# tiems90/mosaic

Hardware: AMD Instinct MI355X
Metric: PIP-join points/sec (H3 res 9) at 1/2/4/8 GPUs + achieved HBM GB/s (higher is better)
Workload: dtype f64

## Files before the change

mosaic_amd/csrc/capi.cpp:

```cpp
#include <hip/hip_runtime.h>

#include <algorithm>
#include <unordered_map>
#include <unordered_set>
#include <chrono>
#include <sched.h>
#include <array>
#include <atomic>
#include <cmath>
#include <cstdarg>
#include <cstdio>
#include <cstring>
#include <cstdlib>
#include <limits>
#include <string>
#include <map>
#include <memory>
#include <functional>
#include <tuple>
#include <mutex>
#include <thread>
#include <vector>

#include "../../include/mosaic_arrow.h"
// ... 1507 lines not shown
  std::vector<uint64_t> ref(ties.size());
  mgpu::parallel_for((int64_t)ties.size(), 256, [&](int64_t b, int64_t e, int) {
    for (int64_t k = b; k < e; k++)
      ref[k] = cells ? mgpu::h3glibc::point_to_cell(ties[k].x, ties[k].y, res)
                     : mgpu::h3glibc::lattice_key(ties[k].x, ties[k].y, res);
  });
  std::vector<std::pair<int64_t, uint64_t>> diff;
  for (size_t k = 0; k < ties.size(); k++)
    if (ref[k] != ties[k].key) diff.push_back({ties[k].pos, ref[k]});
  std::sort(diff.begin(), diff.end());
  return diff;
}

int32_t check_res(int32_t is, int32_t res) {
  if (is == MGPU_H3) {
    if (res < 0 || res > 15) return fail(MGPU_E_RESOLUTION, "H3 resolution has to be between 0 and 15; found %d", res);
    return MGPU_OK;
  }
  if (is == MGPU_BNG) {
    if (res == 0 || res < -6 || res > 6) return fail(MGPU_E_RESOLUTION, "BNG resolution not supported; found %d", res);
    return MGPU_OK;
  }
  return fail(MGPU_E_INVALID_ARG, "unknown index system %d (0 = H3, 1 = BNG)", is);
}

int32_t set_device(int dev) {
  HIP_TRY(hipSetDevice(dev));
  return MGPU_OK;
}

}

extern "C" {

const char* mgpu_last_error(void) { return g_err.c_str(); }
const char* mgpu_version(void) { return "mosaic-mi355x 0.1.0 (gfx950)"; }
int32_t mgpu_join_tile_points(void) { return (int32_t)mgpu::join_tile_points(); }

int32_t mgpu_check_resolution(int32_t index_system, int32_t res) { return check_res(index_system, res); }

int32_t mgpu_ctx_create(int32_t device_id, mgpu_ctx** out) {
  if (!out) return fail(MGPU_E_INVALID_ARG, "out is NULL");
  int n = 0;
  HIP_TRY(hipGetDeviceCount(&n));
  if (device_id < 0 || device_id >= n) return fail(MGPU_E_INVALID_ARG, "device %d not present (%d GPUs)", device_id, n);
  HIP_TRY(hipSetDevice(device_id));
  mgpu_ctx* c = new mgpu_ctx();
  c->device = device_id;
  int32_t st = MGPU_OK;
  if (hipEventCreate(&c->ev0) != hipSuccess || hipEventCreate(&c->ev1) != hipSuccess ||
      hipEventCreate(&c->ev2) != hipSuccess || hipEventCreate(&c->ev3) != hipSuccess ||
      hipHostMalloc((void**)&c->pin, kPinWords * 8, hipHostMallocDefault) != hipSuccess)
    st = fail(MGPU_E_DEVICE, "mgpu_ctx_create: events / pinned page");
  if (!st) st = ensure_ws(c, 1);
  if (!st) st = ensure_tq(c, kTqInit);
  if (st) {
    mgpu_ctx_destroy(c);
    return st;
  }
  *out = c;
  return MGPU_OK;
}

int32_t mgpu_ctx_destroy(mgpu_ctx* ctx) {
  if (!ctx) return MGPU_OK;
  mgpu_comm_destroy(ctx);
  hipSetDevice(ctx->device);
  if (ctx->split_ws) hipFree(ctx->split_ws);
  if (ctx->bin_ws) hipFree(ctx->bin_ws);
  if (ctx->scratch) hipFree(ctx->scratch);
  if (ctx->redo) hipFree(ctx->redo);
  if (ctx->tq) hipFree(ctx->tq);
  if (ctx->ovr) hipFree(ctx->ovr);
  if (ctx->ws) hipFree(ctx->ws);
  if (ctx->pin) hipHostFree(ctx->pin);
  if (ctx->ev0) hipEventDestroy(ctx->ev0);
  if (ctx->ev1) hipEventDestroy(ctx->ev1);
  if (ctx->ev2) hipEventDestroy(ctx->ev2);
  if (ctx->ev3) hipEventDestroy(ctx->ev3);
  delete ctx;
  return MGPU_OK;
}

int32_t mgpu_ctx_set_option(mgpu_ctx* ctx, const char* key, int64_t v) {
  if (!ctx || !key) return fail(MGPU_E_INVALID_ARG, "ctx/key is NULL");
  mgpu_options& o = ctx->opt;
  const std::string k = key;
  auto bad = [&]() { return fail(MGPU_E_INVALID_ARG, "option %s: value %lld out of range", key, (long long)v); };
  if (k == "h3_libm") {
    if (v != MGPU_LIBM_REFERENCE && v != MGPU_LIBM_CORRECTLY_ROUNDED) return bad();
    o.h3_libm = v;
  } else if (k == "pipeline") {
    if (v < MGPU_PIPELINE_AUTO || v > MGPU_PIPELINE_BINNED) return bad();
    o.pipeline = v;
  } else if (k == "bin_count") {
    if (v < 1 || v > mgpu::bin_max()) return bad();
    o.bin_count = v;
  } else if (k == "bin_min_mb") {
    if (v < 0) return bad();
    o.bin_min_mb = v;
  } else if (k == "bin_min_points") {
    if (v < 0) return bad();
    o.bin_min_points = v;
  } else if (k == "bin_xcd") {
    if (v != 0 && v != 1) return bad();
    o.bin_xcd = v;
// ... 1234 lines not shown
    return fail(MGPU_E_INVALID_ARG, "chip table lives on device %d, context on device %d", chips->device, ctx->device);
  if (n < 0 || (n > 0 && (!x || !y))) return fail(MGPU_E_INVALID_ARG, "bad point arrays");
  if (capacity < 0 || (capacity > 0 && (!out_point || !out_poly))) return fail(MGPU_E_INVALID_ARG, "bad output arrays");
  if (int32_t st = set_device(ctx->device)) return st;
  int64_t tiles = mgpu::join_tiles(n);
  const bool emit = count_pool < 0;
  const int64_t pool = emit ? capacity : count_pool;
  if (int32_t st = ensure_ws(ctx, tiles, pool)) return st;
  auto* base = (uint8_t*)ctx->ws;
  const WsLayout L = ws_layout(tiles, pool);
  const mgpu_options& o = ctx->opt;
  mgpu::JoinArgs a;
  a.x = x;
  a.y = y;
  a.n = n;
  a.n_tiles = tiles;
  a.res = res;
  a.res_match = (is == MGPU_BNG || chips->view.res < 0 || chips->view.res == res) ? 1 : 0;
  a.chips = chips->view;
  a.counters = (unsigned long long*)base;
  a.pool_used = a.counters + 5;
  a.n_dirty = (uint32_t*)(a.counters + 6);
  a.dirty = (uint32_t*)(base + L.dirty);
  a.pool_cap = pool;
  a.tile_count = (uint32_t*)(base + L.count);
  a.tile_where = (uint64_t*)(base + L.where);
  a.recs = (uint64_t*)(base + L.recs);
  a.tie_queue = ctx->tq;
  a.tie_cap = ctx->tq_cap;
  a.ovr = ctx->ovr;
  a.n_ovr = n_ovr;
  a.tie_host = (is == MGPU_H3 && tie_host) ? 1 : 0;
  a.pos_of = nullptr;
  mgpu::EmitArgs e;
  e.tile_count = a.tile_count;
  e.group_off = (uint64_t*)(base + L.off);
  a.group_sum = (uint32_t*)(base + L.gsum);
  a.group_cand = a.group_sum + (tiles / 32 + 1);
  e.tile_where = a.tile_where;
  e.recs = a.recs;
  e.point_id = point_id;
  e.id_base = id_base;
  e.capacity = capacity;
  e.out_point = out_point;
  e.out_poly = out_poly;
  a.valid = valid;
  a.valid_off = valid_off;
  a.mixed_idx = nullptr;
  a.mixed_res = nullptr;
  a.chunk_mixed = nullptr;
  a.extra = nullptr;
  a.n_extra = nullptr;
  a.poly_answers = 0;
  HIP_TRY(hipMemsetAsync(base, 0, kWsCounters, s));
  HIP_TRY(hipMemsetAsync(ctx->tq, 0, 16, s));
  const bool bng_grid = is == MGPU_BNG && chips->view.raster_mode == mgpu::kRasterNone &&
                        chips->view.probe_mode == mgpu::kProbeDense && o.bng_split;
  const bool split = (o.pipeline == MGPU_PIPELINE_AUTO || o.pipeline == MGPU_PIPELINE_SPLIT) && n > 0 &&
                     (chips->view.raster_mode != mgpu::kRasterNone || bng_grid) && a.res_match &&
                     (is == MGPU_H3 || res == chips->view.res) && chips->view.max_cell_chips <= 32;
  mgpu::SplitArgs sa{};
  if (split) {
    const int64_t nc = mgpu::split_chunks(n), C = mgpu::split_chunk();
    size_t off = 0;
    auto carve = [&](size_t bytes) {
      const size_t o_ = off;
      off = align_up(off + bytes, 256);
      return o_;
    };
    const size_t o_codes = carve((size_t)nc * C * 4), o_idx = carve((size_t)nc * C * 2), o_res = carve((size_t)nc * C * 8);
    const size_t o_pairs = carve(nc * 4), o_mixed = carve(nc * 4), o_cand = carve(nc * 4), o_off = carve(nc * 8);
    const size_t o_extra = carve((size_t)nc * (C / mgpu::join_tile_points()) * 4);
    if (off > ctx->split_bytes) {
      if (ctx->split_ws) HIP_TRY(hipFree(ctx->split_ws));
      ctx->split_ws = nullptr;
      ctx->split_bytes = 0;
      HIP_TRY(hipMalloc(&ctx->split_ws, off));
      ctx->split_bytes = off;
    }
    auto* sb = (uint8_t*)ctx->split_ws;
    sa.codes = sb + o_codes;
    sa.mixed_idx = (uint16_t*)(sb + o_idx);
    sa.chunk_pairs = (uint32_t*)(sb + o_pairs);
    sa.chunk_mixed = (uint32_t*)(sb + o_mixed);
    sa.chunk_off = (uint64_t*)(sb + o_off);
    a.extra = sa.extra = (uint32_t*)(sb + o_extra);
    a.n_extra = (uint32_t*)(a.counters + 7);
    a.group_sum = sa.chunk_pairs;
    a.group_cand = (uint32_t*)(sb + o_cand);
    a.mixed_idx = sa.mixed_idx;
    a.mixed_res = (uint64_t*)(sb + o_res);
    a.chunk_mixed = sa.chunk_mixed;
    sa.point_id = point_id;
    sa.id_base = id_base;
    sa.capacity = capacity;
    sa.out_point = out_point;
    sa.out_poly = out_poly;
    sa.j = a;
    HIP_TRY(hipMemsetAsync(a.group_cand, 0, nc * 4, s));
  }
  mgpu::BinArgs ba{};
  const bool binned = !split && plan_bins(o, chips, is, res, n, valid, a, ba);
  if (binned) {
    const int64_t nc = mgpu::split_chunks(n), C = mgpu::split_chunk();
    const int64_t K = mgpu::bin_chunks(n), G = mgpu::bin_groups(n), nb = (int64_t)ba.nbx * ba.nby;
    size_t off = 0;
    auto carve = [&](size_t bytes) {
      const size_t o_ = off;
      off = align_up(off + bytes, 256);
      return o_;
    };
    const size_t o_perm = carve((size_t)n * 4), o_rorig = carve((size_t)n * 8);
    const size_t o_bx = carve((size_t)n * 8), o_by = carve((size_t)n * 8),
                 o_pre = carve((size_t)K * nb * 4), o_res = carve((size_t)nc * C * 8), o_cnt = carve((size_t)K * nb * 4),
                 o_gs = carve((size_t)G * nb * 4), o_pairs = carve(nc * 4), o_off = carve(nc * 8),
                 o_gperm = carve(nc * 4), o_gcand = carve(nc * 4);
    const mgpu::ChipTableView& cv = chips->view;
    uint64_t grid_entries = 0;
    for (int f = 0; f < 20; f++) grid_entries = std::max<uint64_t>(grid_entries, (uint64_t)cv.dense[f].base + (uint64_t)cv.dense[f].w * cv.dense[f].h);
    const bool keyed = is == MGPU_H3 && cv.probe_mode == mgpu::kProbeDense && o.bin_keys && grid_entries < (1ull << 30);
    const size_t o_key = keyed ? carve((size_t)n * 4) : 0;
    if (off > ctx->bin_bytes) {
      if (ctx->bin_ws) HIP_TRY(hipFree(ctx->bin_ws));
      ctx->bin_ws = nullptr;
      ctx->bin_bytes = 0;
      HIP_TRY(hipMalloc(&ctx->bin_ws, off));
      ctx->bin_bytes = off;
    }
    auto* bb = (uint8_t*)ctx->bin_ws;
    ba.x = x;
    ba.y = y;
    ba.bx = (double*)(bb + o_bx);
    ba.by = (double*)(bb + o_by);
    ba.pre = (uint32_t*)(bb + o_pre);
    ba.perm = (uint32_t*)(bb + o_perm);
    ba.res = (uint64_t*)(bb + o_rorig);
    ba.cnt = (uint32_t*)(bb + o_cnt);
    ba.gsum = (uint32_t*)(bb + o_gs);
    ba.key = keyed ? (uint32_t*)(bb + o_key) : nullptr;
    mgpu::JoinArgs j = a;
    j.bin_key = ba.key;
    j.x = ba.bx;
    j.y = ba.by;
    j.mixed_idx = nullptr;
    j.chunk_mixed = nullptr;
    j.poly_answers = 1;
    j.pos_of = ba.perm;
    j.mixed_res = (uint64_t*)(bb + o_res);
    j.group_sum = (uint32_t*)(bb + o_gperm);
    j.group_cand = (uint32_t*)(bb + o_gcand);
    ba.s.j = j;
    ba.s.chunk_pairs = (uint32_t*)(bb + o_pairs);
// ... 109 lines not shown
  if (!L.valid || L.binned || (!L.split && pool_used > 0)) return launch_call(ctx, c, timed, n_ovr, 0);
  const int64_t unit = L.split ? mgpu::split_chunk() : mgpu::join_tile_points();
  const int64_t n_units = L.split ? mgpu::split_chunks(L.n) : L.n_tiles;
  std::vector<uint32_t> list;
  for (int64_t p : pos)
    if (list.empty() || list.back() != (uint32_t)(p / unit)) list.push_back((uint32_t)(p / unit));
  if ((int64_t)list.size() * (L.split ? mgpu::split_chunk_tiles() : 1) > L.n_tiles)
    return launch_call(ctx, c, timed, n_ovr, 0);
  const size_t o_aff = 256, o_list = align_up(o_aff + (size_t)n_units, 256), o_old = o_list + list.size() * 4;
  const size_t bytes = o_old + list.size() * 4;
  if (bytes > ctx->redo_bytes) {
    if (ctx->redo) HIP_TRY(hipFree(ctx->redo));
    ctx->redo = nullptr;
    ctx->redo_bytes = 0;
    HIP_TRY(hipMalloc(&ctx->redo, bytes));
    ctx->redo_bytes = bytes;
  }
  auto* rb = (uint8_t*)ctx->redo;
  mgpu::RedoArgs R{(const uint32_t*)(rb + o_list), (uint32_t*)(rb + o_old), rb + o_aff, (uint32_t*)rb,
                   (uint32_t*)(rb + 4)};
  mgpu::JoinArgs a = L.split ? L.sargs.j : L.jargs;
  a.ovr = ctx->ovr;
  a.n_ovr = n_ovr;
  a.tie_host = 0;
  HIP_TRY(hipMemsetAsync(rb, 0, o_list, c.s));
  HIP_TRY(hipMemsetAsync(rb + 4, 0xFF, 4, c.s));
  HIP_TRY(hipMemcpyAsync(rb + o_list, list.data(), list.size() * 4, hipMemcpyHostToDevice, c.s));
  const uint32_t nd = L.split ? 0u : (uint32_t)list.size();
  HIP_TRY(hipMemcpyAsync(a.n_dirty, &nd, 4, hipMemcpyHostToDevice, c.s));
  HIP_TRY(hipStreamSynchronize(c.s));
  if (L.split) {
    mgpu::SplitArgs sa = L.sargs;
    sa.j = a;
    HIP_TRY(mgpu::launch_split_redo(c.is, sa, R, (int64_t)list.size(), c.s, c.count_pool < 0));
    L.sargs = sa;
  } else {
    HIP_TRY(mgpu::launch_join_redo(c.is, a, L.emit, R, (int64_t)list.size(), c.s, c.count_pool < 0));
    L.jargs = a;
  }
  if (timed) HIP_TRY(hipEventRecord(ctx->ev1, c.s));
  if (c.d_n_pairs) HIP_TRY(hipMemcpyAsync(c.d_n_pairs, ctx->ws, 8, hipMemcpyDeviceToDevice, c.s));
  L.n_ovr = n_ovr;
  L.tie_host = 0;
  return MGPU_OK;
}

static int32_t settle_join(mgpu_ctx* ctx, const JoinCall& c, bool timed, bool reference_libm, int64_t* out_n_pairs,
                           mgpu_stats* stats) {
  const hipStream_t s = c.s;
  int64_t n_ovr = 0, n_ties = 0, n_moved = 0;
  int overflows = 0;
  uint64_t h[8] = {0};
  for (;;) {
    HIP_TRY(hipMemcpyAsync(ctx->pin, ctx->ws, 16 * 8, hipMemcpyDeviceToHost, s));
    HIP_TRY(hipMemcpyAsync(ctx->pin + 16, ctx->tq, (2 + 4 * kTqHead) * 8, hipMemcpyDeviceToHost, s));
    HIP_TRY(stream_wait(ctx, s));
    memcpy(h, ctx->pin, sizeof h);
    const int64_t queued = (int64_t)ctx->pin[16];
    if (h[2]) break;
    if (queued > ctx->tq_cap) {
      if (++overflows > 2) return fail(MGPU_E_INTERNAL, "pip_join: the near-tie queue overflowed %d times", overflows);
      if (int32_t e = ensure_tq(ctx, queued + queued / 4 + 1024)) return e;
      if (int32_t e = launch_call(ctx, c, timed, n_ovr, reference_libm && n_ovr == 0)) return e;
      continue;
    }
    if (n_ovr > 0) break;
    n_ties = queued;
    if (!reference_libm || n_ties == 0) break;
    std::vector<TieRec> tr;
    if (int32_t e = read_ties(ctx, n_ties, tr)) return e;
    const auto ref = libm_reference_keys(tr, c.res);
    n_moved = 0;
    for (size_t k = 0; k < tr.size(); k++) n_moved += ref[k].second != tr[k].key;
    if (n_moved == 0) break;
    std::vector<uint64_t> hv(2 * ref.size());
    for (size_t k = 0; k < ref.size(); k++) hv[2 * k] = (uint64_t)ref[k].first, hv[2 * k + 1] = ref[k].second;
    if (int32_t e = ensure_ovr(ctx, (int64_t)hv.size())) return e;
    HIP_TRY(hipMemcpy(ctx->ovr, hv.data(), hv.size() * 8, hipMemcpyHostToDevice));
    n_ovr = (int64_t)ref.size();
    std::vector<int64_t> pos(ref.size());
    for (size_t k = 0; k < ref.size(); k++) pos[k] = (int64_t)ref[k].first;
    if (int32_t e = launch_override_pass(ctx, c, timed, n_ovr, pos, h[5])) return e;
  }
  const int32_t is = c.is;
  const int64_t n = c.n, capacity = c.capacity;
  if (out_n_pairs) *out_n_pairs = (int64_t)h[0];
  if (stats) {
    stats->n_points = n;
    stats->n_pairs = (int64_t)h[0];
    stats->n_near_ties = n_ties;
    stats->n_candidates = (int64_t)h[3];
    stats->libm_overrides = (int32_t)n_moved;
    float ms = 0, ms2 = 0;
    if (timed) {
      hipEventElapsedTime(&ms, ctx->ev0, ctx->ev1);
      if (n > 0) hipEventElapsedTime(&ms2, ctx->ev0, ctx->ev2);
    }
    stats->kernel_ms = ms;
    stats->stream_kernel_ms = ms2;
    stats->mixed_kernel_ms = stats->emit_kernel_ms = 0;
    if (!timed) {
    } else if (ctx->last.split && n > 0) {
      float m3 = 0;
      hipEventElapsedTime(&m3, ctx->ev0, ctx->ev3);
      stats->mixed_kernel_ms = m3 - ms2;
      stats->emit_kernel_ms = ms - m3;
    } else if (ctx->last.binned && n > 0) {
      float m3 = 0;
// ... 667 lines not shown
```

mosaic_amd/csrc/capi_internal.h:

```cpp
#pragma once
#include <hip/hip_runtime.h>
#include <stdint.h>

#include "../../include/mosaic_gpu.h"
#include "chip_table.h"
#include "kernels.h"

struct mgpu_options {
  int64_t h3_libm = MGPU_LIBM_REFERENCE;
  int64_t pipeline = MGPU_PIPELINE_AUTO;
  int64_t bin_count = 64;
  int64_t bin_min_mb = 256;
  int64_t bin_min_points = 1 << 21;
  int64_t bin_xcd = 1;
  int64_t bin_keys = 0;
  int64_t spin_us = 2000;
  int64_t ring_batch = (int64_t)1 << 26;
  int64_t count_lds_slots = 4096;
  int64_t count_groups = 0;
  int64_t kring_batch = 0;
  int64_t bng_split = 0;
  int64_t raster = 1, raster_bng = 0, raster_sub = 16, raster_milli = 250;
};

struct mgpu_ctx {
  int device = 0;
  mgpu_options opt;
  void* ws = nullptr;
  size_t ws_bytes = 0;
  hipEvent_t ev0 = nullptr, ev1 = nullptr, ev2 = nullptr, ev3 = nullptr;
  void* comm = nullptr;
  void* split_ws = nullptr;
  size_t split_bytes = 0;
  void* bin_ws = nullptr;
  size_t bin_bytes = 0;
  uint64_t* tq = nullptr;
  int64_t tq_cap = 0;
  uint64_t* ovr = nullptr;
  int64_t ovr_cap = 0;
  uint64_t* pin = nullptr;
  void* scratch = nullptr;
  size_t scratch_bytes = 0;
  void* redo = nullptr;
  size_t redo_bytes = 0;
  struct {
    bool valid = false, pool_ok = false;
    const mgpu_chips* chips = nullptr;
    int32_t is = 0, res = 0;
    const double *x = nullptr, *y = nullptr;
    const int64_t* point_id = nullptr;
    int64_t id_base = 0, n = 0, total = 0;
    const uint8_t* pts_valid = nullptr;
    int64_t pts_valid_off = 0;
    mgpu::EmitArgs emit{};
    mgpu::JoinArgs jargs{};
    int64_t n_tiles = 0;
    int64_t n_ovr = 0;
    int tie_host = 0;
    bool split = false;
    mgpu::SplitArgs sargs{};
    bool binned = false;
    mgpu::BinArgs bargs{};
    bool async_pending = false;
    int64_t* d_n_pairs = nullptr;
    void* stream = nullptr;
    int64_t capacity = 0;
    int64_t* out_point = nullptr;
    int32_t* out_poly = nullptr;
    int64_t pool = 0, pool_used = 0;
  } last;
};

struct mgpu_chips {
  int device = 0;
  int32_t index_system = MGPU_H3;
  void* blob = nullptr;
  size_t bytes = 0;
  mgpu::ChipTableView view{};
  int64_t n_vertices = 0;
  mutable void* slots = nullptr;
};

namespace mgpu {
int32_t set_error(int32_t code, const char* fmt, ...);
int64_t blob_bytes_of_header(const void* header);
constexpr int64_t kBlobHeaderSize = 1024;
int32_t adopt_device_blob(mgpu_ctx* ctx, void* dev_blob, int64_t bytes, mgpu_chips** out);
}
```

mosaic_amd/csrc/kernels.h:

```cpp
#pragma once
#include <hip/hip_runtime.h>
#include <stdint.h>

#include "../../include/mosaic_gpu.h"
#include "chip_table.h"

namespace mgpu {

struct JoinArgs {
  const double* x;
  const double* y;
  int64_t n;
  int64_t n_tiles;
  int res;
  int res_match;
  ChipTableView chips;
  uint32_t* tile_count;
  uint32_t* group_sum;
  uint32_t* group_cand;
  uint64_t* tile_where;
  uint64_t* recs;
  int64_t pool_cap;
  unsigned long long* pool_used;
  uint32_t* dirty;
// ... 44 lines not shown
};
int64_t split_chunk();
int64_t split_chunk_tiles();
int64_t split_chunks(int64_t n);
hipError_t launch_split(int is, const SplitArgs& a, hipStream_t s, hipEvent_t after_classify, hipEvent_t after_mixed,
                        bool emit = true);
hipError_t launch_split_emit(int is, const SplitArgs& a, hipStream_t s);
hipError_t launch_split_redo(int is, const SplitArgs& sa, const RedoArgs& R, int64_t n, hipStream_t s,
                             bool emit = true);

struct BinArgs {
  SplitArgs s;
  const double* x;
  const double* y;
  double* bx;
  double* by;
  uint32_t* perm;
  uint64_t* res;
  uint32_t* cnt;
  uint32_t* pre;
  uint32_t* gsum;
  double x0, y0, inv_bx, inv_by;
  int32_t nbx, nby;
  int32_t xcd_runs;
  uint32_t* key;
};
int64_t bin_chunk();
int64_t bin_chunks(int64_t n);
int64_t bin_groups(int64_t n);
int32_t bin_max();
hipError_t launch_binned(int is, const BinArgs& a, hipStream_t s, hipEvent_t after_bin, hipEvent_t after_join,
                         bool emit = true);
hipError_t launch_bin_emit(const BinArgs& a, hipStream_t s);

struct EmitArgs {
  const uint32_t* tile_count;
  uint64_t* group_off;
  const uint64_t* tile_where;
  const uint64_t* recs;
  const int64_t* point_id;
  int64_t id_base;
  int64_t capacity;
  int64_t* out_point;
  int32_t* out_poly;
  const uint32_t* redo_first = nullptr;
  const uint8_t* redo_affected = nullptr;
};


hipError_t launch_cells(int is, int res, const double* x, const double* y, int64_t n, int64_t* out,
                        unsigned long long* counters, unsigned long long* ties, int64_t tie_cap,
                        uint64_t* tie_queue, int64_t tq_cap, hipStream_t s, const uint8_t* valid = nullptr,
                        int64_t voff = 0);
hipError_t launch_scatter_i64(const int64_t* pos, const int64_t* val, int64_t n, int64_t* out, hipStream_t s);
hipError_t launch_gather_xy(const double* x, const double* y, const int64_t* pos, int64_t n, double* xy,
                            hipStream_t s);
hipError_t launch_decode_internal(const int32_t* type_id, const int64_t* row_part, const int64_t* part_ring,
                                  const int64_t* ring_off, const double* xy, const uint8_t* valid, int64_t voff,
                                  int64_t n, double* x, double* y, unsigned long long* counters, hipStream_t s);
hipError_t launch_decode_points(int format, const uint8_t* data, const void* offsets, int off32, const uint8_t* valid,
                                int64_t voff, int64_t n, double* x, double* y, unsigned long long* counters,
                                hipStream_t s);
hipError_t launch_valid_and(const uint8_t* a, int64_t aoff, const uint8_t* b, int64_t boff, int64_t n, uint8_t* out,
                            hipStream_t s);
int64_t join_tiles(int64_t n);
int64_t join_tile_points();
int64_t join_slot_records();
hipError_t launch_join(int is, const JoinArgs& a, const EmitArgs& e, hipStream_t s, hipEvent_t after_stream,
                       bool emit = true);
hipError_t launch_join_redo(int is, const JoinArgs& a, const EmitArgs& e, const RedoArgs& R, int64_t n, hipStream_t s,
                            bool emit = true);
hipError_t launch_emit(const EmitArgs& e, int64_t n_tiles, hipStream_t s);

struct CountArgs {
  const int32_t* ids;
  uint32_t n_slots;
  const uint32_t* chip_slot;
  const uint32_t* dense;
  int32_t min_id;
  uint32_t contiguous;
  uint32_t lds_slots;
  uint32_t hash_slots;
  uint32_t stage_n;
  const int64_t* weight;
  unsigned long long* count;
  unsigned long long* sum;
  uint32_t* dropped;
  uint32_t max_groups;
};
constexpr int64_t kCountLdsSlotsMax = 4096;
constexpr int64_t kCountGroupsMax = 65536;
constexpr uint32_t kCountHash = 4096;
constexpr int64_t kCountStageMax = 2048;
hipError_t launch_split_count(int is, const SplitArgs& a, const CountArgs& c, hipStream_t s);
hipError_t launch_tile_count(const EmitArgs& e, int64_t n_tiles, const CountArgs& c, hipStream_t s);
hipError_t launch_bin_count(const BinArgs& b, const CountArgs& c, hipStream_t s);
int64_t format_chunks(int64_t n);
hipError_t launch_format_cells(int is, const int64_t* cells, int64_t n, char* out, int64_t out_bytes,
                               int64_t* offsets, int64_t* chunk, unsigned long long* counters, hipStream_t s);
int64_t format_chunks(int64_t n);
hipError_t launch_kring_count(int is, const int64_t* cells, int64_t n, int k, int loop_only, int64_t* mc,
                              int64_t* chunk, uint32_t* fb_idx, unsigned long long* counters, hipStream_t s);
int64_t kring_fallback_words(int k);
int32_t kring_fallback_max_k();
hipError_t launch_kring_fallback(const int64_t* cells, const uint32_t* fb_idx, int64_t j0, int64_t j1, int k,
                                 int loop_only, int64_t* mc, int64_t* chunk, const int64_t* offsets, int64_t* out,
// ... 9 lines not shown
```

mosaic_amd/csrc/kernels.hip:

```cpp
#include <hip/hip_runtime.h>
#include <stdint.h>

#include <map>
#include <mutex>

#define H3T_QUAL static __constant__ const
#include "h3_core.h"
#include "bng_core.h"
#include "pip_core.h"
#include "h3_ring.h"
#include "kernels.h"
#include "raster.h"

namespace mgpu {

#ifndef MGPU_BLOCK
#define MGPU_BLOCK 64
#endif
constexpr int kBlock = MGPU_BLOCK;
constexpr int kItems = 4;
constexpr int kTile = kBlock * kItems;
constexpr int kStreamBlock = 256;
static_assert(kTile <= 1024, "point-in-tile indices are 10 bits");

// ... 1184 lines not shown
      for (int k = 0; k < kCfyBatch; k++) {
#if MGPU_CFY_ABLATE == 1
        cl[k] = ri[k] < kRasterFull ? (ri[k] & 1) : kPixEmpty;
#elif MGPU_CFY_ABLATE == 2
        cl[k] = ri[k] < kRasterFull && bi[k] != kNoPixel && s_blk[bi[k]] != kPixMixed ? s_blk[bi[k]] : kPixEmpty;
#elif MGPU_CFY_ABLATE == 3
        cl[k] = ri[k] < kRasterFull ? (bi[k] != kNoPixel && s_blk[bi[k]] != kPixMixed ? s_blk[bi[k]] : t.raster[ri[k]])
                                    : kPixEmpty;
#elif MGPU_CFY_ABLATE == 4
        cl[k] = ri[k] < kRasterFull ? t.raster[ri[k]] : kPixEmpty;
#elif MGPU_CFY_ABLATE == 5
        cl[k] = ri[k] < kRasterFull ? (bi[k] != kNoPixel && s_blk[bi[k]] != kPixMixed ? s_blk[bi[k]] : kPixMixed)
                                    : kPixEmpty;
#else
        if (IS == MGPU_BNG && bng_grid)
          cl[k] = ri[k] == kRasterFull ? kPixMixed : (ri[k] == kNoPixel ? kPixEmpty : ri[k]);
        else
          cl[k] = ri[k] < kRasterFull ? raster_class_blk(t, s_blk, ri[k], bi[k], sb[k], s_band)
                                      : (ri[k] == kRasterFull ? kPixMixed : kPixEmpty);
#endif
        if (IS == MGPU_BNG && bng_grid) ge[k] = gix[k];
        else ge[k] = (IS == MGPU_BNG && ri[k] < kRasterFull) ? t.grid[gix[k]] : 0ull;
      }
#pragma unroll
      for (int k = 0; k < kCfyBatch; k++) {
        const int64_t p = c0 + (int64_t)(b + k) * 64 + lane;
        const bool valid = p < a.n;
        bool mixed = cl[k] == kPixMixed;
        Code code;
        if (IS == MGPU_H3) {
          code = (Code)cl[k];
          if (!mixed && cl[k] != kPixEmpty) {
            const uint32_t c = cl[k];
            pairs += c < t.raster_pc[0] ? 1u : c < t.raster_pc[1] ? 2u : c < t.raster_pc[2] ? 3u : c < t.raster_pc[3] ? 4u
                     : (uint32_t)__popc((uint32_t)(t.raster_cls[c] >> 32));
          }
        } else {
          const uint32_t first = (uint32_t)ge[k], m = cl[k];
          if (!mixed && m && !(m < 256u && first < (1u << 24))) mixed = true;
          code = (Code)(mixed ? kCodeMixed32 : (m ? (first << 8) | m : 0u));
          if (!mixed) pairs += __popc(m);
        }
        if (valid) MGPU_ST_INTER(code, &codes[p]);
        mixed = mixed && valid;
        const unsigned long long bal = __ballot(mixed);
        if (mixed) sa.mixed_idx[c0 + nmixed + (uint32_t)__popcll(bal & below)] = (uint16_t)((b + k) * 64 + lane);
        nmixed += (uint32_t)__popcll(bal);
      }
    }
    pairs = wave_sum_u32(pairs);
    if (lane == 0) {
      sa.chunk_pairs[ch] = pairs;
      sa.chunk_mixed[ch] = nmixed;
    }
  }
  count_wave(&a.counters[2], any_bad);
}


#ifndef MGPU_CFY_PAIR
#define MGPU_CFY_PAIR 1
#endif
typedef double dbl2_t __attribute__((ext_vector_type(2)));
template <int IS>
__global__ __launch_bounds__(kCfyBlock) __attribute__((amdgpu_waves_per_eu(MGPU_CFY_WAVES))) void classify_pair_kernel(SplitArgs sa, int64_t n_chunks) {
  using Code = typename CodeOf<IS>::T;
  constexpr int kW = kCfyBlock / 64;
  constexpr int kPairItems = kChunk / 128;
  constexpr int kPB = kCfyBatch / 2 > 0 ? kCfyBatch / 2 : 1;
  constexpr int kPts = 2 * kPB;
  static_assert(kPairItems % kPB == 0, "MGPU_CFY_BATCH / 2 must divide the pair items per lane of a chunk");
  const JoinArgs& a = sa.j;
  const ChipTableView& t = a.chips;
  extern __shared__ uint16_t s_blk[];
  const int lane = threadIdx.x & 63, wave = threadIdx.x >> 6;
  const bool use_blk = IS == MGPU_H3 && t.raster_blk != nullptr;
  const bool bng_grid = IS == MGPU_BNG && t.raster_mode == kRasterNone;
  const uint32_t nblk = use_blk ? t.raster_bnx * t.raster_bny : 0u;
  uint32_t* s_band = (uint32_t*)(s_blk + ((nblk + 1) & ~1u));
  if (use_blk)
    for (uint32_t i = threadIdx.x; i < nblk; i += kCfyBlock) s_blk[i] = t.raster_blk[i];
  if (IS == MGPU_H3)
    for (uint32_t i = threadIdx.x; i < t.raster_nband; i += kCfyBlock) s_band[i] = t.raster_band[i];
  __syncthreads();
  Code* codes = (Code*)sa.codes;
  const unsigned long long below = (1ull << lane) - 1ull;
  bool any_bad = false;
  const int64_t ch_step = (int64_t)gridDim.x * kW;
  for (int64_t ch = (int64_t)blockIdx.x * kW + wave; ch < n_chunks; ch += ch_step) {
    const int64_t c0 = ch * kChunk;
    uint32_t pairs = 0, nmixed = 0;
    for (int b = 0; b < kPairItems; b += kPB) {
      double X[kPts], Y[kPts];
#pragma unroll
      for (int k = 0; k < kPB; k++) {
        const int64_t p = c0 + (int64_t)(b + k) * 128 + 2 * lane;
        if (p + 1 < a.n) {
          const dbl2_t vx = __builtin_nontemporal_load((const dbl2_t*)(a.x + p));
          const dbl2_t vy = __builtin_nontemporal_load((const dbl2_t*)(a.y + p));
          X[2 * k] = vx.x, X[2 * k + 1] = vx.y, Y[2 * k] = vy.x, Y[2 * k + 1] = vy.y;
        } else {
          X[2 * k] = Y[2 * k] = X[2 * k + 1] = Y[2 * k + 1] = 0.0;
          if (p < a.n) X[2 * k] = a.x[p], Y[2 * k] = a.y[p];
        }
      }
      uint32_t ri[kPts], gix[kPts], sb[kPts], bi[kPts];
// ... 31 lines not shown
                                      : (ri[j] == kRasterFull ? kPixMixed : kPixEmpty);
          ge[j] = (IS == MGPU_BNG && ri[j] < kRasterFull) ? t.grid[gix[j]] : 0ull;
        }
      }
      Code code[kPts];
      bool mixed[kPts];
#pragma unroll
      for (int j = 0; j < kPts; j++) {
        const int64_t pj = c0 + (int64_t)(b + j / 2) * 128 + 2 * lane + (j & 1);
        bool m = cl[j] == kPixMixed;
        if (IS == MGPU_H3) {
          code[j] = (Code)cl[j];
          if (!m && cl[j] != kPixEmpty) {
            const uint32_t c = cl[j];
            pairs += c < t.raster_pc[0] ? 1u : c < t.raster_pc[1] ? 2u : c < t.raster_pc[2] ? 3u : c < t.raster_pc[3] ? 4u
                     : (uint32_t)__popc((uint32_t)(t.raster_cls[c] >> 32));
          }
        } else {
          const uint32_t first = (uint32_t)ge[j], mm = cl[j];
          if (!m && mm && !(mm < 256u && first < (1u << 24))) m = true;
          code[j] = (Code)(m ? kCodeMixed32 : (mm ? (first << 8) | mm : 0u));
          if (!m) pairs += __popc(mm);
        }
        mixed[j] = m && pj < a.n;
      }
#pragma unroll
      for (int k = 0; k < kPB; k++) {
        const int64_t p = c0 + (int64_t)(b + k) * 128 + 2 * lane;
        if (p + 1 < a.n) {
          if (sizeof(Code) == 2) {
            MGPU_ST_INTER((uint32_t)code[2 * k] | ((uint32_t)code[2 * k + 1] << 16), (uint32_t*)(codes + p));
          } else {
            typedef uint32_t u32x2_t __attribute__((ext_vector_type(2)));
            u32x2_t v;
            v.x = (uint32_t)code[2 * k];
            v.y = (uint32_t)code[2 * k + 1];
            MGPU_ST_INTER(v, (u32x2_t*)(codes + p));
          }
        } else if (p < a.n) {
          MGPU_ST_INTER(code[2 * k], &codes[p]);
        }
        const unsigned long long b0 = __ballot(mixed[2 * k]), b1 = __ballot(mixed[2 * k + 1]);
        const uint32_t r0 = nmixed + (uint32_t)__popcll(b0 & below) + (uint32_t)__popcll(b1 & below);
        const uint16_t li = (uint16_t)((b + k) * 128 + 2 * lane);
        if (mixed[2 * k]) sa.mixed_idx[c0 + r0] = li;
        if (mixed[2 * k + 1]) sa.mixed_idx[c0 + r0 + (mixed[2 * k] ? 1u : 0u)] = (uint16_t)(li + 1);
        nmixed += (uint32_t)(__popcll(b0) + __popcll(b1));
      }
    }
    pairs = wave_sum_u32(pairs);
    if (lane == 0) {
      sa.chunk_pairs[ch] = pairs;
      sa.chunk_mixed[ch] = nmixed;
    }
  }
  count_wave(&a.counters[2], any_bad);
}

#ifndef MGPU_MIXED_LEAN
#define MGPU_MIXED_LEAN 1
#endif
template <int IS>
__global__ __launch_bounds__(kBlock) MGPU_JOIN_ATTR void pip_mixed_kernel(JoinArgs a) {
  const uint32_t nm = a.chunk_mixed[blockIdx.x];
  if (threadIdx.x == 0 && nm > (uint32_t)kGTile) {
    const uint32_t more = (nm - 1) / kGTile;
    const uint32_t q = atomicAdd(a.n_extra, more);
    for (uint32_t t = 0; t < more; t++) a.extra[q + t] = blockIdx.x * kChunkTiles + 1 + t;
  }
  join_tile<IS, false, 2, MGPU_MIXED_LEAN != 0>(a, blockIdx.x * kChunkTiles);
}

template <int IS>
__global__ __launch_bounds__(kBlock) void pip_mixed_more_kernel(JoinArgs a) {
  const uint32_t n = *a.n_extra;
  for (uint32_t q = blockIdx.x; q < n; q += gridDim.x) {
    join_tile<IS, false, 2>(a, a.extra[q]);
    __syncthreads();
  }
}

template <int IS, int G>
__global__ __launch_bounds__(kBlock) void pip_mixed_fix_kernel(JoinArgs a) {
  const uint32_t nd = *a.n_dirty;
  for (uint32_t q = blockIdx.x; q < nd; q += gridDim.x) {
    join_tile<IS, true, G>(a, a.dirty[q]);
    __syncthreads();
  }
}

#ifndef MGPU_EMIT_LDSBAR
#define MGPU_EMIT_LDSBAR 1
#endif
__device__ __forceinline__ void lds_barrier() {
#if MGPU_EMIT_LDSBAR
  asm volatile("s_waitcnt lgkmcnt(0)\n\ts_barrier" ::: "memory");
#else
  __syncthreads();
#endif
}

__device__ __forceinline__ uint32_t chunk_excl_scan(uint32_t v, uint32_t* s_w, uint32_t* total) {
  const int lane = threadIdx.x & 63, wave = threadIdx.x >> 6;
  const uint32_t incl = wave_incl_scan(v);
  if (lane == 63) s_w[wave] = incl;
  lds_barrier();
// ... 140 lines not shown
        bool has_one = false;
        int32_t one = 0;
        if (c == kMixed) {
          const uint32_t rr = r++;
          v = mres(rr);
          if (rr < kMr && __popc((uint32_t)(v >> 32)) == 1)
            has_one = true, one = (int32_t)(uint32_t)v, v = 0;
        } else if (IS == MGPU_H3 && c != 0 && (uint32_t)c < ncp)
          has_one = true, one = s_cp[(uint32_t)c];
        else if (c != 0)
          v = pure(c);
        if (has_one) {
          if (q >= w0 && q < w0 + kEmitWin) {
            s_poly[emit_swz(q - w0)] = (uint32_t)one;
            s_pt[emit_swz(q - w0)] = (uint16_t)(threadIdx.x * kClsItems + k);
          }
          q++;
        }
        const uint32_t first = (uint32_t)v;
        for (uint32_t m = (uint32_t)(v >> 32); m; m &= m - 1, q++)
          if (q >= w0 && q < w0 + kEmitWin) {
            s_poly[emit_swz(q - w0)] = (uint32_t)t.chip_poly[first + __builtin_ctz(m)];
            s_pt[emit_swz(q - w0)] = (uint16_t)(threadIdx.x * kClsItems + k);
          }
      }
    }
    lds_barrier();
    const uint32_t cnt = total - w0 < (uint32_t)kEmitWin ? total - w0 : (uint32_t)kEmitWin;
    for (uint32_t i = threadIdx.x; i < cnt; i += kClsBlock) {
      const uint64_t q = base + w0 + i;
      if ((int64_t)q >= sa.capacity) break;
      const int64_t p = c0 + s_pt[emit_swz(i)];
#if MGPU_EMIT_NT
      __builtin_nontemporal_store(sa.point_id ? sa.point_id[p] : sa.id_base + p, &sa.out_point[q]);
      __builtin_nontemporal_store((int32_t)s_poly[emit_swz(i)], &sa.out_poly[q]);
#else
      sa.out_point[q] = sa.point_id ? sa.point_id[p] : sa.id_base + p;
      sa.out_poly[q] = (int32_t)s_poly[emit_swz(i)];
#endif
    }
    lds_barrier();
  }
}

constexpr int kScanBlock = 1024;
constexpr int kScanLds = 24576;
__global__ __launch_bounds__(kScanBlock) void tile_scan_kernel(const uint32_t* __restrict__ gsum,
                                                               const uint32_t* __restrict__ gcand, int64_t ng,
                                                               uint64_t* __restrict__ goff,
                                                               unsigned long long* __restrict__ counters,
                                                               const uint32_t* only_if = nullptr) {
  if (only_if && *only_if == 0) return;
  __shared__ unsigned long long s_w[kScanBlock / 64];
  __shared__ uint32_t s_v[kScanLds];
  __shared__ unsigned long long s_base[kScanBlock];
  const int lane = threadIdx.x & 63, wave = threadIdx.x >> 6;
  const int64_t per = (ng + kScanBlock - 1) / kScanBlock;
  const int64_t b = threadIdx.x * per, e = b + per < ng ? b + per : ng;
  unsigned long long cand = 0, sum = 0;
  const bool lds = ng <= kScanLds;
  if (lds) {
    for (int64_t i = threadIdx.x; i < ng; i += kScanBlock) {
      cand += gcand[i];
      s_v[i] = gsum[i];
    }
    __syncthreads();
    for (int64_t i = b; i < e; i++) sum += s_v[i];
  } else {
    for (int64_t i = b; i < e; i++) {
      cand += gcand[i];
      sum += gsum[i];
    }
  }
  cand = wave_sum_u64(cand);
  if (lane == 0 && cand) atomicAdd(&counters[3], cand);
  unsigned long long incl = sum;
#pragma unroll
  for (int d = 1; d < 64; d <<= 1) {
    const unsigned long long u = __shfl_up(incl, d, 64);
    if (lane >= d) incl += u;
  }
  if (lane == 63) s_w[wave] = incl;
  __syncthreads();
  unsigned long long run = incl - sum, tot = 0;
  for (int w = 0; w < kScanBlock / 64; w++) {
    if (w < wave) run += s_w[w];
    tot += s_w[w];
  }
  if (lds) {
    s_base[threadIdx.x] = run;
    uint32_t rel = 0;
    for (int64_t i = b; i < e; i++) {
      const uint32_t v = s_v[i];
      s_v[i] = rel;
      rel += v;
    }
    __syncthreads();
    for (int64_t i = threadIdx.x; i < ng; i += kScanBlock) goff[i] = s_base[i / per] + s_v[i];
  } else {
    for (int64_t i = b; i < e; i++) {
      goff[i] = run;
      run += gsum[i];
    }
  }
  if (threadIdx.x == 0) counters[0] = tot;
}

constexpr int kEmitBlock = 256;
constexpr int kEmitTiles = 4096 / kTile;
static_assert(kScanGroup % kEmitTiles == 0 && kEmitTiles <= 64, "emit groups inside scan groups");
__global__ __launch_bounds__(kEmitBlock) void pair_emit_kernel(EmitArgs a, int64_t n_tiles) {
  __shared__ uint32_t s_pref[kEmitTiles + 1];
  __shared__ uint64_t s_where[kEmitTiles];
  __shared__ int64_t s_off;
  const int64_t t0 = (int64_t)blockIdx.x * kEmitTiles;
  if (a.redo_affected && t0 + kEmitTiles <= (int64_t)*a.redo_first) {
    bool any = false;
    for (int k = 0; k < kEmitTiles && t0 + k < n_tiles; k++) any |= a.redo_affected[t0 + k] != 0;
    if (!any) return;
  }
  if (threadIdx.x < 64) {
    const int lane = threadIdx.x;
    const int64_t t = t0 + lane;
    const bool in = lane < kEmitTiles && t < n_tiles;
    const uint32_t cnt = in ? a.tile_count[t] : 0u;
    if (lane < kEmitTiles) s_where[lane] = in ? a.tile_where[t] : kNoDst;
    const uint32_t incl = wave_incl_scan(cnt);
    if (lane < kEmitTiles) s_pref[lane + 1] = incl;
    if (lane == 0) s_pref[0] = 0;
    const int64_t g0 = t0 - t0 % kScanGroup;
    const int64_t j = g0 + lane;
    unsigned long long v = (lane < kScanGroup && j < t0) ? a.tile_count[j] : 0u;
    v = wave_sum_u64(v);
    if (lane == 0) s_off = (int64_t)(a.group_off[t0 / kScanGroup] + v);
  }
  __syncthreads();
  const int64_t off = s_off;
  const uint32_t total = s_pref[kEmitTiles];
  for (uint32_t i = threadIdx.x; i < total; i += kEmitBlock) {
    const int64_t q = off + i;
    if (q >= a.capacity) break;
    int k = 0;
#pragma unroll
    for (int step = kEmitTiles / 2; step >= 1; step >>= 1)
      if (s_pref[k + step] <= i) k += step;
    const uint64_t where = s_where[k];
    if (where == kNoDst) continue;
    const uint64_t r = a.recs[where + (i - s_pref[k])];
    const int64_t p = (t0 + k) * kTile + (int64_t)(r >> 32);
#if MGPU_EMIT_NT_OTHER
    __builtin_nontemporal_store(a.point_id ? a.point_id[p] : a.id_base + p, &a.out_point[q]);
// ... 831 lines not shown
        for (uint32_t mm = msk; mm; mm &= mm - 1, q++)
          if (q >= w0 && q < w0 + kEmitWin) {
            s_poly[emit_swz(q - w0)] = (uint32_t)t.chip_poly[first + __builtin_ctz(mm)];
            s_pt[emit_swz(q - w0)] = (uint16_t)(l0 + i);
          }
      }
    }
    __syncthreads();
    const uint32_t cnt = total - w0 < (uint32_t)kEmitWin ? total - w0 : (uint32_t)kEmitWin;
    for (uint32_t i = threadIdx.x; i < cnt; i += kBinBlock) {
      const uint64_t q = base + w0 + i;
      if ((int64_t)q >= sa.capacity) break;
      const int64_t p = c0 + s_pt[emit_swz(i)];
      sa.out_point[q] = sa.point_id ? sa.point_id[p] : sa.id_base + p;
      sa.out_poly[q] = (int32_t)s_poly[emit_swz(i)];
    }
    __syncthreads();
  }
}

__global__ __launch_bounds__(256) void scatter_i64_kernel(const int64_t* __restrict__ pos, const int64_t* __restrict__ val,
                                                          int64_t n, int64_t* __restrict__ out) {
  for (int64_t k = (int64_t)blockIdx.x * 256 + threadIdx.x; k < n; k += (int64_t)gridDim.x * 256) out[pos[k]] = val[k];
}

__global__ __launch_bounds__(256) void gather_xy_kernel(const double* __restrict__ x, const double* __restrict__ y,
                                                        const int64_t* __restrict__ pos, int64_t n,
                                                        double* __restrict__ xy) {
  for (int64_t k = (int64_t)blockIdx.x * 256 + threadIdx.x; k < n; k += (int64_t)gridDim.x * 256) {
    xy[2 * k] = x[pos[k]];
    xy[2 * k + 1] = y[pos[k]];
  }
}


hipError_t launch_cells(int is, int res, const double* x, const double* y, int64_t n, int64_t* out,
                        unsigned long long* counters, unsigned long long* ties, int64_t tie_cap, uint64_t* tie_queue,
                        int64_t tq_cap, hipStream_t s, const uint8_t* valid, int64_t voff) {
  if (n <= 0) return hipSuccess;
  int64_t blocks = (n + kStreamBlock - 1) / kStreamBlock;
  if (blocks > 256 * 64) blocks = 256 * 64;
  if (is == MGPU_H3) {
    hipLaunchKernelGGL(cells_kernel<MGPU_H3>, dim3((unsigned)blocks), dim3(kStreamBlock), 0, s, x, y, n, res, out, counters,
                       ties, tie_cap, valid, voff);
    hipLaunchKernelGGL(cells_fix_kernel, dim3(256), dim3(kStreamBlock), 0, s, x, y, n, res, out, counters, ties, tie_cap,
                       tie_queue, tq_cap, valid, voff);
  } else {
    hipLaunchKernelGGL(cells_kernel<MGPU_BNG>, dim3((unsigned)blocks), dim3(kStreamBlock), 0, s, x, y, n, res, out,
                       counters, ties, tie_cap, valid, voff);
  }
  return hipGetLastError();
}

hipError_t launch_scatter_i64(const int64_t* pos, const int64_t* val, int64_t n, int64_t* out, hipStream_t s) {
  if (n <= 0) return hipSuccess;
  const int64_t blocks = std::min<int64_t>((n + 255) / 256, 1024);
  hipLaunchKernelGGL(scatter_i64_kernel, dim3((unsigned)blocks), dim3(256), 0, s, pos, val, n, out);
  return hipGetLastError();
}

hipError_t launch_gather_xy(const double* x, const double* y, const int64_t* pos, int64_t n, double* xy, hipStream_t s) {
  if (n <= 0) return hipSuccess;
  const int64_t blocks = std::min<int64_t>((n + 255) / 256, 1024);
  hipLaunchKernelGGL(gather_xy_kernel, dim3((unsigned)blocks), dim3(256), 0, s, x, y, pos, n, xy);
  return hipGetLastError();
}

__global__ __launch_bounds__(kStreamBlock) void valid_and_kernel(const uint8_t* __restrict__ a, int64_t aoff,
                                                               const uint8_t* __restrict__ b, int64_t boff, int64_t n,
                                                               uint8_t* __restrict__ out) {
  const int64_t byte = (int64_t)blockIdx.x * blockDim.x + threadIdx.x;
  if (byte * 8 >= n) return;
  uint8_t v = 0;
  for (int k = 0; k < 8; k++) {
    const int64_t p = byte * 8 + k;
    if (p < n && pt_valid(a, aoff, p) && pt_valid(b, boff, p)) v |= (uint8_t)(1u << k);
  }
  out[byte] = v;
}

hipError_t launch_valid_and(const uint8_t* a, int64_t aoff, const uint8_t* b, int64_t boff, int64_t n, uint8_t* out,
                            hipStream_t s) {
  if (n <= 0) return hipSuccess;
  const int64_t bytes = (n + 7) / 8;
  hipLaunchKernelGGL(valid_and_kernel, dim3((unsigned)((bytes + kStreamBlock - 1) / kStreamBlock)), dim3(kStreamBlock), 0,
                     s, a, aoff, b, boff, n, out);
  return hipGetLastError();
}

int64_t join_tiles(int64_t n) { return (n + kTile - 1) / kTile; }
int64_t join_tile_points() { return kTile; }
int64_t join_slot_records() { return kSlot; }

#ifndef MGPU_FIX_GRID
#define MGPU_FIX_GRID 8192
#endif
constexpr int64_t kFixGrid = MGPU_FIX_GRID;
hipError_t launch_join(int is, const JoinArgs& a, const EmitArgs& e, hipStream_t s, hipEvent_t after_stream, bool emit) {
  if (a.n_tiles <= 0) return hipSuccess;
  const unsigned fix_blocks = (unsigned)(a.n_tiles < kFixGrid ? a.n_tiles : kFixGrid);
  if (is == MGPU_H3) {
    hipLaunchKernelGGL(pip_join_kernel<MGPU_H3>, dim3((unsigned)a.n_tiles), dim3(kBlock), 0, s, a);
    if (after_stream) hipEventRecord(after_stream, s);
    hipLaunchKernelGGL(pip_fix_kernel<MGPU_H3>, dim3(fix_blocks), dim3(kBlock), 0, s, a);
  } else {
    hipLaunchKernelGGL(pip_join_kernel<MGPU_BNG>, dim3((unsigned)a.n_tiles), dim3(kBlock), 0, s, a);
// ... 252 lines not shown
```

Measured before the change: 104.5 billion.

## Replace join memsets and readback memcpys with tiny kernels; pad scan LDS

The two per-join hipMemsetAsync calls are replaced by a single one-block clear kernel. The group_cand zeroing moves into the chunk kernels that already write per-chunk counts. The two device-to-host counter readback copies become one kernel that writes directly into the mapped pinned page through its device pointer and ends with a system fence. Separately, the group scan kernel's LDS layout is padded with an odd stride so each thread's contiguous run avoids bank conflicts. The aim is to cut per-call launch and DMA overhead on small joins; the cost is reliance on host-mapped coherent memory plus extra LDS.

```diff
diff --git a/mosaic_amd/csrc/capi.cpp b/mosaic_amd/csrc/capi.cpp
--- a/mosaic_amd/csrc/capi.cpp
+++ b/mosaic_amd/csrc/capi.cpp
@@ -1583,6 +1583,8 @@
       hipEventCreate(&c->ev2) != hipSuccess || hipEventCreate(&c->ev3) != hipSuccess ||
       hipHostMalloc((void**)&c->pin, kPinWords * 8, hipHostMallocDefault) != hipSuccess)
     st = fail(MGPU_E_DEVICE, "mgpu_ctx_create: events / pinned page");
+  if (!st && hipHostGetDevicePointer((void**)&c->pin_dev, c->pin, 0) != hipSuccess)
+    st = fail(MGPU_E_DEVICE, "mgpu_ctx_create: the pinned page is not device-visible");
   if (!st) st = ensure_ws(c, 1);
   if (!st) st = ensure_tq(c, kTqInit);
   if (st) {
@@ -2923,8 +2925,8 @@
   a.extra = nullptr;
   a.n_extra = nullptr;
   a.poly_answers = 0;
-  HIP_TRY(hipMemsetAsync(base, 0, kWsCounters, s));
-  HIP_TRY(hipMemsetAsync(ctx->tq, 0, 16, s));
+  static_assert(kWsCounters == mgpu::kCounterWords * 8, "launch_join_clear clears the counters");
+  HIP_TRY(mgpu::launch_join_clear(a.counters, ctx->tq, s));
   const bool bng_grid = is == MGPU_BNG && chips->view.raster_mode == mgpu::kRasterNone &&
                         chips->view.probe_mode == mgpu::kProbeDense && o.bng_split;
   const bool split = (o.pipeline == MGPU_PIPELINE_AUTO || o.pipeline == MGPU_PIPELINE_SPLIT) && n > 0 &&
@@ -2968,7 +2970,6 @@
     sa.out_point = out_point;
     sa.out_poly = out_poly;
     sa.j = a;
-    HIP_TRY(hipMemsetAsync(a.group_cand, 0, nc * 4, s));
   }
   mgpu::BinArgs ba{};
   const bool binned = !split && plan_bins(o, chips, is, res, n, valid, a, ba);
@@ -3184,8 +3185,8 @@
   int overflows = 0;
   uint64_t h[8] = {0};
   for (;;) {
-    HIP_TRY(hipMemcpyAsync(ctx->pin, ctx->ws, 16 * 8, hipMemcpyDeviceToHost, s));
-    HIP_TRY(hipMemcpyAsync(ctx->pin + 16, ctx->tq, (2 + 4 * kTqHead) * 8, hipMemcpyDeviceToHost, s));
+    static_assert(kPinWords == mgpu::kCounterWords + 2 + 4 * kTqHead, "launch_join_readback fills the pinned page");
+    HIP_TRY(mgpu::launch_join_readback((const unsigned long long*)ctx->ws, ctx->tq, (int)(2 + 4 * kTqHead), ctx->pin_dev, s));
     HIP_TRY(stream_wait(ctx, s));
     memcpy(h, ctx->pin, sizeof h);
     const int64_t queued = (int64_t)ctx->pin[16];
diff --git a/mosaic_amd/csrc/capi_internal.h b/mosaic_amd/csrc/capi_internal.h
--- a/mosaic_amd/csrc/capi_internal.h
+++ b/mosaic_amd/csrc/capi_internal.h
@@ -39,6 +39,7 @@
   uint64_t* ovr = nullptr;
   int64_t ovr_cap = 0;
   uint64_t* pin = nullptr;
+  uint64_t* pin_dev = nullptr;
   void* scratch = nullptr;
   size_t scratch_bytes = 0;
   void* redo = nullptr;
diff --git a/mosaic_amd/csrc/kernels.h b/mosaic_amd/csrc/kernels.h
--- a/mosaic_amd/csrc/kernels.h
+++ b/mosaic_amd/csrc/kernels.h
@@ -120,6 +120,10 @@
                         unsigned long long* counters, unsigned long long* ties, int64_t tie_cap,
                         uint64_t* tie_queue, int64_t tq_cap, hipStream_t s, const uint8_t* valid = nullptr,
                         int64_t voff = 0);
+constexpr int kCounterWords = 16;
+hipError_t launch_join_clear(unsigned long long* counters, uint64_t* tie_queue, hipStream_t s);
+hipError_t launch_join_readback(const unsigned long long* counters, const uint64_t* tie_queue, int tq_words,
+                                uint64_t* pin, hipStream_t s);
 hipError_t launch_scatter_i64(const int64_t* pos, const int64_t* val, int64_t n, int64_t* out, hipStream_t s);
 hipError_t launch_gather_xy(const double* x, const double* y, const int64_t* pos, int64_t n, double* xy,
                             hipStream_t s);
diff --git a/mosaic_amd/csrc/kernels.hip b/mosaic_amd/csrc/kernels.hip
--- a/mosaic_amd/csrc/kernels.hip
+++ b/mosaic_amd/csrc/kernels.hip
@@ -1260,6 +1260,7 @@
     if (lane == 0) {
       sa.chunk_pairs[ch] = pairs;
       sa.chunk_mixed[ch] = nmixed;
+      a.group_cand[ch] = 0;
     }
   }
   count_wave(&a.counters[2], any_bad);
@@ -1397,6 +1398,7 @@
     if (lane == 0) {
       sa.chunk_pairs[ch] = pairs;
       sa.chunk_mixed[ch] = nmixed;
+      a.group_cand[ch] = 0;
     }
   }
   count_wave(&a.counters[2], any_bad);
@@ -1643,20 +1645,27 @@
                                                                const uint32_t* only_if = nullptr) {
   if (only_if && *only_if == 0) return;
   __shared__ unsigned long long s_w[kScanBlock / 64];
-  __shared__ uint32_t s_v[kScanLds];
+  __shared__ uint32_t s_v[kScanLds + kScanBlock];
   __shared__ unsigned long long s_base[kScanBlock];
   const int lane = threadIdx.x & 63, wave = threadIdx.x >> 6;
   const int64_t per = (ng + kScanBlock - 1) / kScanBlock;
   const int64_t b = threadIdx.x * per, e = b + per < ng ? b + per : ng;
   unsigned long long cand = 0, sum = 0;
   const bool lds = ng <= kScanLds;
+  const uint32_t per32 = lds && per > 0 ? (uint32_t)per : 1u, stride = per32 | 1u;
+  const uint32_t q0 = threadIdx.x / per32, j0 = threadIdx.x % per32;
+  const uint32_t dq = (uint32_t)kScanBlock / per32, dr = (uint32_t)kScanBlock % per32;
+  const uint32_t run0 = threadIdx.x * stride, nrun = (uint32_t)(e > b ? e - b : 0);
   if (lds) {
-    for (int64_t i = threadIdx.x; i < ng; i += kScanBlock) {
+    uint32_t q = q0, j = j0;
+    for (uint32_t i = threadIdx.x; i < (uint32_t)ng; i += kScanBlock) {
       cand += gcand[i];
-      s_v[i] = gsum[i];
+      s_v[q * stride + j] = gsum[i];
+      q += dq, j += dr;
+      if (j >= per32) j -= per32, q++;
     }
     __syncthreads();
-    for (int64_t i = b; i < e; i++) sum += s_v[i];
+    for (uint32_t k = 0; k < nrun; k++) sum += s_v[run0 + k];
   } else {
     for (int64_t i = b; i < e; i++) {
       cand += gcand[i];
@@ -1681,13 +1690,18 @@
   if (lds) {
     s_base[threadIdx.x] = run;
     uint32_t rel = 0;
-    for (int64_t i = b; i < e; i++) {
-      const uint32_t v = s_v[i];
-      s_v[i] = rel;
+    for (uint32_t k = 0; k < nrun; k++) {
+      const uint32_t v = s_v[run0 + k];
+      s_v[run0 + k] = rel;
       rel += v;
     }
     __syncthreads();
-    for (int64_t i = threadIdx.x; i < ng; i += kScanBlock) goff[i] = s_base[i / per] + s_v[i];
+    uint32_t q = q0, j = j0;
+    for (uint32_t i = threadIdx.x; i < (uint32_t)ng; i += kScanBlock) {
+      goff[i] = s_base[q] + s_v[q * stride + j];
+      q += dq, j += dr;
+      if (j >= per32) j -= per32, q++;
+    }
   } else {
     for (int64_t i = b; i < e; i++) {
       goff[i] = run;
@@ -2625,6 +2639,31 @@
   return hipGetLastError();
 }
 
+__global__ __launch_bounds__(64) void join_clear_kernel(unsigned long long* __restrict__ counters,
+                                                        uint64_t* __restrict__ tie_queue) {
+  if (threadIdx.x < kCounterWords) counters[threadIdx.x] = 0;
+  else if (threadIdx.x < kCounterWords + 2) tie_queue[threadIdx.x - kCounterWords] = 0;
+}
+
+__global__ __launch_bounds__(256) void join_readback_kernel(const unsigned long long* __restrict__ counters,
+                                                            const uint64_t* __restrict__ tie_queue, int tq_words,
+                                                            uint64_t* __restrict__ pin) {
+  for (int i = threadIdx.x; i < kCounterWords + tq_words; i += 256)
+    pin[i] = i < kCounterWords ? (uint64_t)counters[i] : tie_queue[i - kCounterWords];
+  __threadfence_system();
+}
+
+hipError_t launch_join_clear(unsigned long long* counters, uint64_t* tie_queue, hipStream_t s) {
+  hipLaunchKernelGGL(join_clear_kernel, dim3(1), dim3(64), 0, s, counters, tie_queue);
+  return hipGetLastError();
+}
+
+hipError_t launch_join_readback(const unsigned long long* counters, const uint64_t* tie_queue, int tq_words,
+                                uint64_t* pin, hipStream_t s) {
+  hipLaunchKernelGGL(join_readback_kernel, dim3(1), dim3(256), 0, s, counters, tie_queue, tq_words, pin);
+  return hipGetLastError();
+}
+
 hipError_t launch_scatter_i64(const int64_t* pos, const int64_t* val, int64_t n, int64_t* out, hipStream_t s) {
   if (n <= 0) return hipSuccess;
   const int64_t blocks = std::min<int64_t>((n + 255) / 256, 1024);
```

Result: faster. 106.5 billion (median of 6 runs) (+1.9%).
